# mohwald/gandtr

Hardware: AMD Instinct MI355X
Metric: images/sec generator@256^2 + descriptors/sec GeM-R101@1024^2, 1/2/4/8 MI355X (higher is better)
Workload: dtype f16c; 1 GPU; cyclegan ResnetGenerator 9-block (InstanceNorm) forward, synthetic 3x256x256, random-init weights; batch_per_gpu=64, global_batch=64, parallelism=dp1

## Files before the change

gandtr_amd/csrc/conv3x3_halo_c16.hip:

```cpp
#include <cstdio>
#include <cstdlib>

#include <vector>

#ifdef GDT_C_STAMP
#define GDT_STAMP_ON
#endif
#include "conv_device.h"

#ifndef GDT_C16_ABL
#define GDT_C16_ABL 0
#endif

namespace {

constexpr int ROWB = 128;
constexpr int QROWB = 64;
constexpr int HW_ = 18, HROWS = HW_ * HW_, HROWS_PAD = 328;
constexpr int A_BYTES = HROWS_PAD * ROWB;
constexpr int Q_BYTES = HROWS_PAD * QROWB;
constexpr int STAGE_BYTES = A_BYTES + Q_BYTES;
constexpr int NORM_BYTES = 4096 + 64;
constexpr int E_OFF = 2 * STAGE_BYTES + NORM_BYTES;
constexpr size_t LDS_BYTES = 2 * (size_t)STAGE_BYTES + NORM_BYTES + 2 * HROWS_PAD;
constexpr int NT = 256, RPR = NT / 8, NR = (HROWS_PAD + RPR - 1) / RPR;
constexpr int NTAP = 9, SLOTS = NTAP * 3;
constexpr int SPR = 2;
#ifndef GDT_C16_SDIST
#define GDT_C16_SDIST 2
#endif
constexpr int SDIST = GDT_C16_SDIST;
static_assert((NR + SDIST) * SPR <= SLOTS, "halo rounds are spread over the slots of the previous chunk");

__device__ __forceinline__ void mfma16(f32x4& acc, const f16x8& a, const f16x8& b) {
    asm volatile("v_mfma_f32_16x16x32_f16 %0, %1, %2, %0" : "+a"(acc) : "v"(a), "v"(b) : "memory");
}
__device__ __forceinline__ void mfma16_mx(f32x4& acc, const v6i& a6, const v4i& b4, int sa, int sb) {
    asm volatile("v_mfma_scale_f32_16x16x128_f8f6f4 %0, %1, %2, %0, %3, %4 op_sel_hi:[0,0,0] cbsz:2 blgp:4" : "+a"(acc) : "v"(a6), "v"(b4), "v"(sa), "v"(sb) : "memory");
}
__device__ __forceinline__ float gdt_max3_abs(float a, float b, float c) {
    float m;
    asm("v_max3_f32 %0, |%1|, |%2|, |%3|" : "=v"(m) : "v"(a), "v"(b), "v"(c));
    return m;
}
__device__ __forceinline__ float gdt_max_abs(float a, float b) {
    float m;
    asm("v_max_f32_e64 %0, |%1|, |%2|" : "=v"(m) : "v"(a), "v"(b));
    return m;
}

template <int MODE>
__global__ __launch_bounds__(NT) void conv3x3_halo_c16_kernel(const ConvLaunch d, const int vblocks) {
    constexpr bool NORM = (MODE & 1) != 0, RES = (MODE & 2) != 0, WB = (MODE & 4) != 0;
    constexpr int RING = 3;
    static_assert(18 % RING == 0, "ring slot of a half-step must not depend on the chunk");
    constexpr int AW = 8, QW = 4;
    extern __shared__ __attribute__((aligned(16))) char smem[];

    const int tid = threadIdx.x, lane = tid & 63;
    const int wave = __builtin_amdgcn_readfirstlane(tid >> 6);
    const float* __restrict__ inf = (const float*)d.in;
    const float* __restrict__ resf = (const float*)d.in_res;
    float* __restrict__ wbf = (float*)d.in_out;

    const int tiles_x = d.W >> 4, tiles_y = d.H >> 4;
    const int tpi = tiles_x * tiles_y, ntm = d.N * tpi, ntn = d.CoutPad >> 8;
    auto tile_at = [&](int vb) -> GdtPatch { return gdt_patch_at(vb, vblocks, ntm, ntn, tpi, tiles_x, 16); };
    int vb = blockIdx.x;
    GdtPatch cur = tile_at(vb);
    if (!cur.valid) return;

    const int lrow = tid >> 3;
    const bool refl = d.pad_reflect != 0;
    struct Pend { float4 r0, r1, s0, s1; unsigned goff; bool ok; };
    auto load_piece = [&](const GdtPatch& ta, int chunk, int r) -> Pend {
        int lr = lrow;
        asm volatile("" : "+v"(lr));
        const int h = min(r * RPR + lr, HROWS_PAD - 1);
        int hy, hx;
        gdt_halo_yx<HW_>(h, hy, hx);
        const int q = lane & 7;
        const int iy = ta.y0 - 1 + hy, ix = ta.x0 - 1 + hx;
        const int cbyte = (chunk * 8 + q) * 32;
        int ry, rx;
        GDT_REFLECT_CLAMP(iy, ix, d.H, d.W, ry, rx)
        const bool inb = ((unsigned)iy < (unsigned)d.H) & ((unsigned)ix < (unsigned)d.W);
        Pend p;
        p.goff = (((unsigned)((ta.n * d.H + ry) * d.W + rx) << (d.lc8 + 5)) + cbyte);
        p.ok = (h < HROWS) & (inb | refl);
        p.r0 = *(const float4*)((const char*)inf + p.goff); p.r1 = *(const float4*)((const char*)inf + p.goff + 16);
        if (RES) { p.s0 = *(const float4*)((const char*)resf + p.goff); p.s1 = *(const float4*)((const char*)resf + p.goff + 16); }
        return p;
    };
    Pend pendv[SDIST];
    float* nlds = (float*)(smem + 2 * STAGE_BYTES);
    auto stage_norm = [&](const GdtPatch& ta, int slot) {
        gdt_stage_norm(nlds, slot, d.in_norm, d.Cin, ta.n, tid, NT);
    };
    float4 nf[4];
    auto load_nf = [&](int slot, int chunk) {
        if (!NORM) return;
        const float4* np4 = (const float4*)(nlds + slot * 512 + (chunk * 8 + (lane & 7)) * 16);
#pragma unroll
        for (int k = 0; k < 4; ++k) nf[k] = np4[k];
    };
    auto store_piece = [&](int stage_off, int r, const Pend& p) {
        const int row = min(r * RPR + lrow, HROWS_PAD - 1);
        int phy, phx;
        gdt_halo_yx<HW_>(row, phy, phx);
        float a[8] = {p.r0.x, p.r0.y, p.r0.z, p.r0.w, p.r1.x, p.r1.y, p.r1.z, p.r1.w};
        if (NORM) {
            const float lo = d.in_relu ? 0.f : -3.0e38f;
#pragma unroll
            for (int k = 0; k < 4; ++k) {
                const float4 v = nf[k];
                a[2 * k] = fmaxf(fmaf(a[2 * k], v.x, v.y), lo);
                a[2 * k + 1] = fmaxf(fmaf(a[2 * k + 1], v.z, v.w), lo);
            }
            if (RES) {
                a[0] += p.s0.x; a[1] += p.s0.y; a[2] += p.s0.z; a[3] += p.s0.w;
                a[4] += p.s1.x; a[5] += p.s1.y; a[6] += p.s1.z; a[7] += p.s1.w;
            }
        }
        if (WB) {
            *(float4*)((char*)wbf + p.goff) = make_float4(a[0], a[1], a[2], a[3]);
            *(float4*)((char*)wbf + p.goff + 16) = make_float4(a[4], a[5], a[6], a[7]);
        }
#pragma unroll
        for (int e = 0; e < 8; ++e) a[e] = p.ok ? a[e] : 0.f;
        const int ex = gdt_c_pixel_exp(a);
        const float lo_scale = gdt_exp2i(ex - 13), hi_scale = gdt_exp2i(ex - 2);
        unsigned ou[4], qlo = 0, qhi = 0;
        gdt_c_split<0>(a[0], a[1], lo_scale, hi_scale, ou[0], qlo, qhi);
        gdt_c_split<1>(a[2], a[3], lo_scale, hi_scale, ou[1], qlo, qhi);
        gdt_c_split<2>(a[4], a[5], lo_scale, hi_scale, ou[2], qlo, qhi);
        gdt_c_split<3>(a[6], a[7], lo_scale, hi_scale, ou[3], qlo, qhi);
        const u32x4 ov = {ou[0], ou[1], ou[2], ou[3]};
        const int q = lane & 7;
        *(f16x8*)(smem + stage_off + row * ROWB + ((q ^ ((phx >> 1) & 7)) << 4)) = __builtin_bit_cast(f16x8, ov);
        const int key2 = (phx >> 2) & 3;
        const int qo = stage_off + A_BYTES + row * QROWB + ((((q >> 2) << 1) ^ key2) << 4) + ((q & 3) << 2);
        *(unsigned*)(smem + qo) = qlo;
        *(unsigned*)(smem + (qo ^ 16)) = qhi;
        smem[E_OFF + (stage_off ? HROWS_PAD : 0) + row] = (char)(127 + ex - 13);
    };

    float sa[8];
    unsigned sou[4], sqlo = 0, sqhi = 0;
    int sex = 0;
    float slo_scale = 1.f, shi_scale = 1.f;
    int mh = 0, mt = 0, my = 0, mx = 0, ma = 0, mb = 0;
    int wrow = 0, wx = 0, wa = 0, wq = 0;
    float mu = 0.f, ml0 = 0.f, ml1 = 0.f;
    int mbits = 0;
    int gy0 = 0, gx0 = 0;
    int wes = E_OFF + HROWS_PAD;
    auto stage_micro = [&](const GdtPatch& ta, int chunk, int stage_off, int sl, int row, int g) {
        if (GDT_C16_ABL & 1) return;
        const int r = sl / SPR, mp = ((sl % SPR) * 16 + row) * 2 + g;
        const bool st = r >= SDIST && r - SDIST < NR, ld = r < NR;
        Pend& pend = pendv[r % SDIST];
        constexpr int P_NORM = 0, P_RES = P_NORM + (NORM ? 8 : 1), P_WB = P_RES + (NORM && RES ? 3 : 0), P_MASK = P_WB + (WB ? 2 : 0), P_MAX = P_MASK + 3,
                      P_DPP = P_MAX + 2, P_EXP = P_DPP + 3, P_SPLIT = P_EXP + 2, P_ADDR = P_SPLIT + 10, P_WRITE = P_ADDR + 7, P_GADDR = P_WRITE + 4,
                      P_LOAD = P_GADDR + 9, P_END = P_LOAD + (RES ? 4 : 2);
        static_assert(P_END <= SPR * 16 * 2, "a round's micro-phases fit the positions of its slot pair");
#define GDT_PIN1(a) asm volatile("" : "+v"(a))
#define GDT_PIN2(a, b) asm volatile("" : "+v"(a), "+v"(b))
#define GDT_PIN3(a, b, c) asm volatile("" : "+v"(a), "+v"(b), "+v"(c))
#define GDT_PIN4(a, b, c, e) asm volatile("" : "+v"(a), "+v"(b), "+v"(c), "+v"(e))
        auto f4 = [](float4& v, int i) -> float& { return i == 0 ? v.x : (i == 1 ? v.y : (i == 2 ? v.z : v.w)); };
        auto pr = [&](int e) -> float& { return e < 4 ? f4(pend.r0, e) : f4(pend.r1, e - 4); };
        auto ps = [&](int e) -> float& { return e < 4 ? f4(pend.s0, e) : f4(pend.s1, e - 4); };
        if (st && !NORM && mp == P_NORM) {
#pragma unroll
            for (int e = 0; e < 8; ++e) sa[e] = pr(e);
            GDT_PIN4(sa[0], sa[1], sa[2], sa[3]); GDT_PIN4(sa[4], sa[5], sa[6], sa[7]);
        }
        if (st && NORM && mp >= P_NORM && mp < P_NORM + 8) {
            const int e = mp - P_NORM;
            const float lo = d.in_relu ? 0.f : -3.0e38f;
            const float4 v = nf[e >> 1];
            float x = pr(e);
            GDT_PIN1(x);
            x = fmaxf(fmaf(x, (e & 1) ? v.z : v.x, (e & 1) ? v.w : v.y), lo);
            GDT_PIN1(x);
            sa[e] = x;
        }
        if (st && NORM && RES && mp >= P_RES && mp < P_RES + 3) {
            const int e = 3 * (mp - P_RES);
            float y0 = ps(e), y1 = ps(e + 1), y2 = ps(e + 2 < 8 ? e + 2 : e);
            if (e + 2 < 8) { GDT_PIN3(sa[e], sa[e + 1], sa[e + 2]); GDT_PIN3(y0, y1, y2); } else { GDT_PIN2(sa[e], sa[e + 1]); GDT_PIN2(y0, y1); }
            sa[e] += y0; sa[e + 1] += y1;
            if (e + 2 < 8) { sa[e + 2] += y2; GDT_PIN3(sa[e], sa[e + 1], sa[e + 2]); } else GDT_PIN2(sa[e], sa[e + 1]);
        }
        if (st && WB && mp == P_WB) {
            GDT_PIN4(sa[0], sa[1], sa[2], sa[3]);
            *(float4*)((char*)wbf + pend.goff) = make_float4(sa[0], sa[1], sa[2], sa[3]);
        }
        if (st && WB && mp == P_WB + 1) {
            GDT_PIN4(sa[4], sa[5], sa[6], sa[7]);
            *(float4*)((char*)wbf + pend.goff + 16) = make_float4(sa[4], sa[5], sa[6], sa[7]);
        }
        if (st && mp >= P_MASK && mp < P_MASK + 3) {
            const int e = 3 * (mp - P_MASK);
            if (e + 2 < 8) GDT_PIN3(sa[e], sa[e + 1], sa[e + 2]); else GDT_PIN2(sa[e], sa[e + 1]);
            sa[e] = pend.ok ? sa[e] : 0.f; sa[e + 1] = pend.ok ? sa[e + 1] : 0.f;
            if (e + 2 < 8) { sa[e + 2] = pend.ok ? sa[e + 2] : 0.f; GDT_PIN3(sa[e], sa[e + 1], sa[e + 2]); } else GDT_PIN2(sa[e], sa[e + 1]);
        }
        if (st && mp == P_MAX) {
            GDT_PIN4(sa[0], sa[1], sa[2], sa[3]); GDT_PIN1(sa[4]);
            mu = gdt_max3_abs(gdt_max3_abs(sa[0], sa[1], sa[2]), sa[3], sa[4]);
            GDT_PIN1(mu);
        }
        if (st && mp == P_MAX + 1) {
            GDT_PIN4(mu, sa[5], sa[6], sa[7]);
            mu = gdt_max_abs(gdt_max3_abs(mu, sa[5], sa[6]), sa[7]);
            mbits = __float_as_int(mu);
            sqlo = 0; sqhi = 0;
            GDT_PIN3(mbits, sqlo, sqhi);
        }
        if (st && mp >= P_DPP && mp < P_DPP + 3) {
            GDT_PIN1(mbits);
            if (mp == P_DPP) mbits = max(mbits, __builtin_amdgcn_mov_dpp(mbits, 0xB1, 0xF, 0xF, false));
            if (mp == P_DPP + 1) mbits = max(mbits, __builtin_amdgcn_mov_dpp(mbits, 0x4E, 0xF, 0xF, false));
            if (mp == P_DPP + 2) mbits = max(mbits, __builtin_amdgcn_mov_dpp(mbits, 0x141, 0xF, 0xF, false));
            GDT_PIN1(mbits);
        }
        if (st && mp == P_EXP) {
            GDT_PIN1(mbits);
            sex = min(max(mbits >> 23, 127 - 14), 127 + 15);
            GDT_PIN1(sex);
        }
        if (st && mp == P_EXP + 1) {
            GDT_PIN1(sex);
            slo_scale = __int_as_float((sex - 13) << 23); shi_scale = __int_as_float((sex - 2) << 23);
            GDT_PIN2(slo_scale, shi_scale);
        }
        if (st && mp >= P_SPLIT && mp < P_SPLIT + 10) {
            GDT_PIN4(sqlo, sqhi, ml0, ml1);
#pragma unroll
            for (int i = 2 * (mp - P_SPLIT); i < 2 * (mp - P_SPLIT) + 2; ++i) {
                const int K = i / 5, w = i - 5 * K;
                GDT_PIN2(sa[2 * K], sa[2 * K + 1]);
                if (w > 0) GDT_PIN1(sou[K]);
                if (w == 0) sou[K] = gdt_pk_f16(sa[2 * K], sa[2 * K + 1]);
                if (w == 1) asm("v_fma_mix_f32 %0, -%1, 1.0, %2 op_sel:[0,0,0] op_sel_hi:[1,0,0]" : "=v"(ml0) : "v"(sou[K]), "v"(sa[2 * K]));
                if (w == 2) asm("v_fma_mix_f32 %0, -%1, 1.0, %2 op_sel:[1,0,0] op_sel_hi:[1,0,0]" : "=v"(ml1) : "v"(sou[K]), "v"(sa[2 * K + 1]));
                if (w == 3) {
                    GDT_PIN1(shi_scale);
                    if (K == 0) sqhi = __builtin_amdgcn_cvt_scalef32_pk_fp4_f16(sqhi, __builtin_bit_cast(f16x2, sou[K]), shi_scale, 0);
                    if (K == 1) sqhi = __builtin_amdgcn_cvt_scalef32_pk_fp4_f16(sqhi, __builtin_bit_cast(f16x2, sou[K]), shi_scale, 1);
                    if (K == 2) sqhi = __builtin_amdgcn_cvt_scalef32_pk_fp4_f16(sqhi, __builtin_bit_cast(f16x2, sou[K]), shi_scale, 2);
                    if (K == 3) sqhi = __builtin_amdgcn_cvt_scalef32_pk_fp4_f16(sqhi, __builtin_bit_cast(f16x2, sou[K]), shi_scale, 3);
                }
                if (w == 4) {
                    GDT_PIN1(slo_scale);
                    if (K == 0) sqlo = __builtin_amdgcn_cvt_scalef32_pk_fp4_f32(sqlo, ml0, ml1, slo_scale, 0);
                    if (K == 1) sqlo = __builtin_amdgcn_cvt_scalef32_pk_fp4_f32(sqlo, ml0, ml1, slo_scale, 1);
                    if (K == 2) sqlo = __builtin_amdgcn_cvt_scalef32_pk_fp4_f32(sqlo, ml0, ml1, slo_scale, 2);
                    if (K == 3) sqlo = __builtin_amdgcn_cvt_scalef32_pk_fp4_f32(sqlo, ml0, ml1, slo_scale, 3);
                }
                GDT_PIN1(sou[K]);
            }
            GDT_PIN4(sqlo, sqhi, ml0, ml1);
        }
        const int q = lane & 7;
        if (st && mp == P_ADDR) {
            int lr = lrow;
            GDT_PIN1(lr);
            wrow = min((r - SDIST) * RPR + lr, HROWS_PAD - 1);
            GDT_PIN1(wrow);
        }
        if (st && mp == P_ADDR + 1) {
            GDT_PIN1(wrow);
            wx = wrow - ((wrow * (65536 / HW_ + 1)) >> 16) * HW_;
            GDT_PIN1(wx);
        }
        if (st && mp == P_ADDR + 2) {
            GDT_PIN1(wx);
            wa = q ^ ((wx >> 1) & 7);
            GDT_PIN1(wa);
        }
        if (st && mp == P_ADDR + 3) {
            GDT_PIN2(wrow, wa);
            wa = stage_off + wrow * ROWB + (wa << 4);
            GDT_PIN1(wa);
        }
        if (st && mp == P_ADDR + 4) {
            GDT_PIN1(wx);
            wx = ((q >> 2) << 1) ^ ((wx >> 2) & 3);
            GDT_PIN1(wx);
        }
        if (st && mp == P_ADDR + 5) {
            GDT_PIN1(wx);
            wq = (wx << 4) + ((q & 3) << 2);
            GDT_PIN1(wq);
        }
        if (st && mp == P_ADDR + 6) {
            GDT_PIN2(wrow, wq);
            wq = stage_off + A_BYTES + wrow * QROWB + wq;
            GDT_PIN1(wq);
        }
        if (st && mp == P_WRITE) {
            GDT_PIN1(wa); GDT_PIN4(sou[0], sou[1], sou[2], sou[3]);
            const u32x4 ov = {sou[0], sou[1], sou[2], sou[3]};
            *(f16x8*)(smem + wa) = __builtin_bit_cast(f16x8, ov);
        }
        if (st && mp == P_WRITE + 1) {
            GDT_PIN2(wq, sqlo);
            *(unsigned*)(smem + wq) = sqlo;
        }
        if (st && mp == P_WRITE + 2) {
            GDT_PIN2(wq, sqhi);
            *(unsigned*)(smem + (wq ^ 16)) = sqhi;
        }
        if (st && mp == P_WRITE + 3) {
            GDT_PIN2(wrow, sex);
            smem[wes + wrow] = (char)(sex - 13);
        }
        if (ld && mp == P_GADDR) {
            int lr = lrow;
            GDT_PIN1(lr);
            mh = min(r * RPR + lr, HROWS_PAD - 1);
            GDT_PIN1(mh);
        }
        if (ld && mp == P_GADDR + 1) {
            GDT_PIN1(mh);
            mt = (mh * (65536 / HW_ + 1)) >> 16;
            GDT_PIN2(mh, mt);
        }
        if (ld && mp == P_GADDR + 2) {
            GDT_PIN2(mh, mt);
            my = gy0 + mt; mx = gx0 + (mh - mt * HW_);
            GDT_PIN3(mh, my, mx);
        }
        if (ld && mp == P_GADDR + 3) {
            GDT_PIN3(mh, my, mx);
            const bool inb = ((unsigned)my < (unsigned)d.H) & ((unsigned)mx < (unsigned)d.W);
            pend.ok = (mh < HROWS) & (inb | refl);
        }
        if (ld && mp == P_GADDR + 4) {
            GDT_PIN1(my);
            ma = max(my, -my); mb = 2 * d.H - 2 - ma;
            GDT_PIN2(ma, mb);
        }
        if (ld && mp == P_GADDR + 5) {
            GDT_PIN2(ma, mb);
            my = min(max(min(ma, mb), 0), d.H - 1);
            GDT_PIN1(my);
        }
        if (ld && mp == P_GADDR + 6) {
            GDT_PIN1(mx);
            ma = max(mx, -mx); mb = 2 * d.W - 2 - ma;
            GDT_PIN2(ma, mb);
        }
        if (ld && mp == P_GADDR + 7) {
            GDT_PIN2(ma, mb);
            mx = min(max(min(ma, mb), 0), d.W - 1);
            GDT_PIN1(mx);
        }
        if (ld && mp == P_GADDR + 8) {
            GDT_PIN2(my, mx);
            pend.goff = (((unsigned)((ta.n * d.H + my) * d.W + mx) << (d.lc8 + 5)) + (chunk * 8 + q) * 32);
            GDT_PIN1(pend.goff);
        }
        if (ld && mp == P_LOAD) pend.r0 = *(const float4*)((const char*)inf + pend.goff);
        if (ld && mp == P_LOAD + 1) pend.r1 = *(const float4*)((const char*)inf + pend.goff + 16);
        if (ld && RES && mp == P_LOAD + 2) pend.s0 = *(const float4*)((const char*)resf + pend.goff);
        if (ld && RES && mp == P_LOAD + 3) pend.s1 = *(const float4*)((const char*)resf + pend.goff + 16);
#undef GDT_PIN1
#undef GDT_PIN2
#undef GDT_PIN3
#undef GDT_PIN4
    };

    auto wgrp = [&](int tile_n) -> long { return (long)tile_n * 4 + wave; };
    const int nms = d.Kpad >> 6, cin64 = d.Cin >> 6;
    f16x8 bw[RING][4];
    constexpr int BQ_MFMA = (GDT_C16_ABL & 64) ? 1 : 0;
    v6i bq[1 + BQ_MFMA][4];
    v4i bqs[1 + BQ_MFMA];
    auto lane_bytes = [&](int per_lane) -> unsigned {
        unsigned v = lane * per_lane;
        asm volatile("" : "+v"(v));
        return v;
    };
    unsigned lo16 = lane_bytes(16), lo8 = lane_bytes(8), lo4 = lane_bytes(4);
    constexpr long WREC = 15360;
    auto load_bw = [&](int rs, int cb, int tile_n, long ks) {
        const char* wb = (const char*)d.w_c16 + (unsigned)(((tile_n * 4 + wave) * nms + (int)(ks >> 1)) * (int)WREC + (int)(ks & 1) * 4096);
        bw[rs][cb] = *(const f16x8*)(wb + lo16 + cb * 1024);
    };
    auto load_bq_part = [&](int set, int part, int tile_n, long ms) {
        const long f0 = (GDT_C16_ABL & 128) ? 0 : wgrp(tile_n) * nms + ms;
        const char* rec = (const char*)d.w_c16 + (unsigned)((int)f0 * (int)WREC);
        const int cb = part >> 1;
        if (part == 8) bqs[set] = *(const v4i*)(rec + 14336 + lo16);
        else if ((part & 1) == 0) {
            const v4i qa = *(const v4i*)(rec + 8192 + lo16 + cb * 1024);
            bq[set][cb] = __builtin_shufflevector(__builtin_shufflevector(qa, qa, 0, 1, 2, 3, -1, -1), bq[set][cb], 0, 1, 2, 3, 10, 11);
        } else {
            const v2i qb = *(const v2i*)(rec + 12288 + lo8 + cb * 512);
            bq[set][cb] = __builtin_shufflevector(bq[set][cb], __builtin_shufflevector(qb, qb, 0, 1, -1, -1, -1, -1), 0, 1, 2, 3, 6, 7);
        }
    };

    const int fn = lane & 15, fg = lane >> 4;
    const int px = fn < 4 ? 2 * fn : (fn < 12 ? 2 * (fn - 4) + 1 : 2 * (fn - 8));
    int vt[3], vq[3];
#pragma unroll
    for (int tx = 0; tx < 3; ++tx) {
        vt[tx] = px * ROWB + ((fg ^ (((px + tx) >> 1) & 7)) << 4);
        vq[tx] = A_BYTES + px * QROWB + ((fg ^ (((px + tx) >> 2) & 3)) << 4);
    }
    auto a_frag = [&](int pb, int ty, int tx, int s) -> f16x8 {
        return *(const f16x8*)(smem + (vt[tx] ^ (s << 6)) + ((pb + ty) * HW_ + tx) * ROWB);
    };
    auto a_qfrag = [&](int pb, int ty, int tx) -> v4i {
        return *(const v4i*)(smem + vq[tx] + ((pb + ty) * HW_ + tx) * QROWB);
    };
    int ve = E_OFF + px;
    auto a_efrag = [&](int pb, int ty, int tx) -> int {
        return *(const unsigned char*)(smem + ve + (pb + ty) * HW_ + tx);
    };
    auto flip_stage = [&](int delta) {
        ve += delta > 0 ? HROWS_PAD : -HROWS_PAD;
        wes -= delta > 0 ? HROWS_PAD : -HROWS_PAD;
#pragma unroll
        for (int k = 0; k < 3; ++k) { vt[k] += delta; vq[k] += delta; }
    };
    const int a_scale_off = (fg & 1) ? GDT_C_HI_SCALE_OFF : 0;
    constexpr bool AE_PRE = !(GDT_C16_ABL & (2 | 8));

    const int nchunks = d.Cin >> 6;
#pragma unroll
    for (int u = 0; u < RING - 1; ++u)
#pragma unroll
        for (int cb = 0; cb < 4; ++cb) load_bw(u, cb, cur.tile_n, u);
    if (NORM) {
        stage_norm(cur, 0);
        __syncthreads();
    }
    load_nf(0, 0);
#pragma unroll
    for (int r = 0; r < NR; ++r) store_piece(0, r, load_piece(cur, 0, r));
    __syncthreads();
#pragma unroll
    for (int k = 0; k < SDIST; ++k) pendv[k] = load_piece(cur, 0, 0);

    f16x8 afr[AW];
    v4i aq[QW];
    int ae[QW];
    if (GDT_C16_ABL & 8) { for (int i = 0; i < QW; ++i) { aq[i] = a_qfrag(i, 0, 0); ae[i] = a_efrag(i, 0, 0); } }
    if (GDT_C16_ABL & (16 | 64)) { for (int st = 0; st < 1 + BQ_MFMA; ++st) for (int part = 0; part < 9; ++part) load_bq_part(st, part, cur.tile_n, 0); }
#pragma unroll
    for (int i = 0; i < AW; ++i) afr[i] = a_frag(i, 0, 0, 0);

    int so = 0;
    int slot = 0;
#ifdef GDT_C_STAMP
    unsigned long long st_body = 0, st_cbar = 0, st_tbar = 0, st_epi = 0, st_t = __builtin_amdgcn_s_memtime(), st_n = 0;
    const unsigned long long st_begin = st_t;
#endif
    for (;;) {
        const GdtPatch nxt = tile_at(vb + gridDim.x);
        f32x4 acc[16][4];
#pragma unroll
        for (int i = 0; i < 16; ++i)
#pragma unroll
            for (int j = 0; j < 4; ++j)
#pragma unroll
                for (int e = 0; e < 4; ++e) acc[i][j][e] = 0.f;

        for (int c = 0; c < nchunks; ++c) {
            const bool last = c + 1 == nchunks;
            const bool to_next = last && nxt.valid;
            const GdtPatch sta = to_next ? nxt : cur;
            const int sc = last ? 0 : c + 1, sslot = to_next ? slot ^ 1 : slot;
            if (NORM && nxt.valid && c == nchunks - 2) stage_norm(nxt, slot ^ 1);
            load_nf(sslot, sc);
            lo16 = lane_bytes(16); lo8 = lane_bytes(8); lo4 = lane_bytes(4);
            auto ks_of = [&](int u) -> long { return u < 18 ? (long)(((u >> 1) * cin64 + c) * 2 + (u & 1)) : (long)(sc * 2 + (u - 18)); };
            auto tn_of = [&](int u) -> int { return (u >= 18 && last) ? nxt.tile_n : cur.tile_n; };
            gy0 = sta.y0 - 1; gx0 = sta.x0 - 1;
            asm volatile("" : "+s"(gy0), "+s"(gx0));
            __builtin_amdgcn_sched_barrier(0);
#pragma unroll
            for (int t = 0; t < NTAP; ++t) {
                const int ty = t / 3, tx = t - ty * 3;
                const int nty = (t + 1) / 3, ntx = (t + 1) - nty * 3;
#pragma unroll
                for (int s = 0; s < 2; ++s) {
                    const int u = 2 * t + s;
#pragma unroll
                    for (int pb = 0; pb < 16; ++pb) {
#pragma unroll
                        for (int cb = 0; cb < 4; ++cb) {
                            mfma16(acc[pb][cb], bw[u % RING][cb], afr[pb % AW]);
                            if (cb == 0) {
                                if (AE_PRE && s == 1 && pb == 15) { asm volatile("" : "+v"(ae[0])); ae[0] += a_scale_off; asm volatile("" : "+v"(ae[0])); }
                                if (!(GDT_C16_ABL & 4) && (pb & 3) == 2) load_bw((u + RING - 1) % RING, pb >> 2, tn_of(u + RING - 1), ks_of(u + RING - 1));
                                if (!(GDT_C16_ABL & (2 | 16)) && (pb & 1) == 1 && (s == 0 || pb == 1)) load_bq_part(0, s == 0 ? pb >> 1 : 8, cur.tile_n, (long)(t * cin64 + c));
                            } else if (cb < 3) {
                                stage_micro(sta, sc, STAGE_BYTES - so, 3 * t + s, pb, cb - 1);
                            } else {
                                if (pb + AW < 16) afr[pb % AW] = a_frag(pb + AW, ty, tx, s);
                                else if (s == 0) afr[pb % AW] = a_frag(pb + AW - 16, ty, tx, 1);
                                else if (t < NTAP - 1) afr[pb % AW] = a_frag(pb + AW - 16, nty, ntx, 0);
                                if (!(GDT_C16_ABL & (2 | 8)) && s == 1 && pb >= 16 - QW) { aq[pb - (16 - QW)] = a_qfrag(pb - (16 - QW), ty, tx); ae[pb - (16 - QW)] = a_efrag(pb - (16 - QW), ty, tx); }
                            }
                            __builtin_amdgcn_sched_barrier(0);
                        }
                    }
                }
#pragma unroll
                for (int pb = 0; pb < 16; ++pb) {
#pragma unroll
                    for (int cb = 0; cb < 4; ++cb) {
                        if (!(GDT_C16_ABL & 2)) {
                            mfma16_mx(acc[pb][cb], bq[BQ_MFMA][cb], aq[pb % QW], bqs[BQ_MFMA][cb], AE_PRE ? ae[pb % QW] : ae[pb % QW] + a_scale_off);
                            if (cb == 0 && AE_PRE && pb + 1 < 16) { asm volatile("" : "+v"(ae[(pb + 1) % QW])); ae[(pb + 1) % QW] += a_scale_off; asm volatile("" : "+v"(ae[(pb + 1) % QW])); }
                            if (cb == 3 && !(GDT_C16_ABL & 8) && pb + QW < 16) { aq[pb % QW] = a_qfrag(pb + QW, ty, tx); ae[pb % QW] = a_efrag(pb + QW, ty, tx); }
                        }
                        if (cb == 1 || cb == 2) stage_micro(sta, sc, STAGE_BYTES - so, 3 * t + 2, pb, cb - 1);
                        __builtin_amdgcn_sched_barrier(0);
                    }
                }
            }
            if (GDT_C16_ABL & 64) {
#pragma unroll
                for (int cb = 0; cb < 4; ++cb) asm volatile("" :: "v"(bq[0][cb]));
                asm volatile("" :: "v"(bqs[0]));
            }
            GDT_STAMP(st_body)
            if (!last) {
                asm volatile("s_waitcnt lgkmcnt(0)" ::: "memory");
                __builtin_amdgcn_s_barrier();
                asm volatile("" ::: "memory");
                GDT_STAMP(st_cbar)
                flip_stage(STAGE_BYTES - 2 * so);
                so = STAGE_BYTES - so;
#pragma unroll
                for (int i = 0; i < AW; ++i) afr[i] = a_frag(i, 0, 0, 0);
            }
        }

        asm volatile("s_waitcnt lgkmcnt(0)" ::: "memory");
        __builtin_amdgcn_s_barrier();
        asm volatile("" ::: "memory");
        GDT_STAMP(st_tbar)
        const int so_next = STAGE_BYTES - so;

        {
            float* __restrict__ outp = (float*)d.out;
            const float* __restrict__ resp = (const float*)d.res;
            int lane_e = lane;
            asm volatile("" : "+v"(lane_e));
            const int n_e = lane_e & 15, g_e = lane_e >> 4;
            const int x_e = n_e < 4 ? 2 * n_e : (n_e < 12 ? 2 * (n_e - 4) + 1 : 2 * (n_e - 8));
            const int ch = cur.tile_n * 256 + wave * 64 + 4 * g_e;
            unsigned o = (unsigned)((cur.n * d.H + cur.y0) * d.W + cur.x0 + x_e) * (unsigned)d.Cout + (unsigned)ch;
            const unsigned rowstep = (unsigned)d.W * (unsigned)d.Cout;
            const bool lowhalf = n_e < 8;
            const int n_p = n_e ^ 8, x_p = n_p < 4 ? 2 * n_p : (n_p < 12 ? 2 * (n_p - 4) + 1 : 2 * (n_p - 8));
            const unsigned o_p = o + (unsigned)((x_p - x_e) * d.Cout);
            unsigned oA = (lowhalf ? o : o_p) + (lowhalf ? 0u : 16u), oB = (lowhalf ? o_p : o) + (lowhalf ? 0u : 16u);
            const float lo = d.relu ? 0.f : -__builtin_inff();
            constexpr bool EPI_RES = MODE == 0;
            const bool has_res = EPI_RES && resp != nullptr;
            float4 bv[4], s1[4], s2[4];
#pragma unroll
            for (int cb = 0; cb < 4; ++cb) {
                bv[cb] = d.bias ? *(const float4*)(d.bias + ch + cb * 16) : make_float4(0.f, 0.f, 0.f, 0.f);
                s1[cb] = make_float4(0.f, 0.f, 0.f, 0.f); s2[cb] = make_float4(0.f, 0.f, 0.f, 0.f);
            }
            float4 rcur[4], rnxt[4];
            if (has_res) {
#pragma unroll
                for (int cb = 0; cb < 4; ++cb) rcur[cb] = *(const float4*)(resp + o + cb * 16);
            }
#pragma unroll
            for (int pb = 0; pb < 16; ++pb) {
                asm volatile("" : "+v"(o));
                if (has_res && pb + 1 < 16) {
#pragma unroll
                    for (int cb = 0; cb < 4; ++cb) rnxt[cb] = *(const float4*)(resp + o + rowstep + cb * 16);
                }
                float4 tv[4];
#pragma unroll
                for (int cb = 0; cb < 4; ++cb) {
                    const f32x4& a = acc[pb][cb];
                    float4 t = make_float4(a[0] + bv[cb].x, a[1] + bv[cb].y, a[2] + bv[cb].z, a[3] + bv[cb].w);
                    s1[cb].x += t.x; s1[cb].y += t.y; s1[cb].z += t.z; s1[cb].w += t.w;
                    s2[cb].x += t.x * t.x; s2[cb].y += t.y * t.y; s2[cb].z += t.z * t.z; s2[cb].w += t.w * t.w;
                    if (has_res) { t.x += rcur[cb].x; t.y += rcur[cb].y; t.z += rcur[cb].z; t.w += rcur[cb].w; }
                    t.x = fmaxf(t.x, lo); t.y = fmaxf(t.y, lo); t.z = fmaxf(t.z, lo); t.w = fmaxf(t.w, lo);
                    tv[cb] = t;
                }
                if (GDT_C16_ABL & 256) {
#pragma unroll
                    for (int cb = 0; cb < 4; ++cb) asm volatile("" :: "v"(tv[cb].x), "v"(tv[cb].y), "v"(tv[cb].z), "v"(tv[cb].w));
                } else {
                    auto ror8 = [](float v) -> float { return __builtin_bit_cast(float, __builtin_amdgcn_update_dpp(0, __builtin_bit_cast(int, v), 0x128, 0xf, 0xf, false)); };
#pragma unroll
                    for (int p2 = 0; p2 < 2; ++p2) {
                        const float4 t0 = tv[2 * p2], t1 = tv[2 * p2 + 1];
                        const float rx = ror8(lowhalf ? t1.x : t0.x), ry = ror8(lowhalf ? t1.y : t0.y), rz = ror8(lowhalf ? t1.z : t0.z), rw = ror8(lowhalf ? t1.w : t0.w);
                        *(float4*)(outp + oA + p2 * 32) = make_float4(lowhalf ? t0.x : rx, lowhalf ? t0.y : ry, lowhalf ? t0.z : rz, lowhalf ? t0.w : rw);
                        *(float4*)(outp + oB + p2 * 32) = make_float4(lowhalf ? rx : t1.x, lowhalf ? ry : t1.y, lowhalf ? rz : t1.z, lowhalf ? rw : t1.w);
                    }
                    oA += rowstep; oB += rowstep;
                }
                o += rowstep;
                if (has_res) {
#pragma unroll
                    for (int cb = 0; cb < 4; ++cb) rcur[cb] = rnxt[cb];
                }
            }
            if (d.stats) {
                auto merge = [](float v) -> float {
                    v += __builtin_bit_cast(float, __builtin_amdgcn_update_dpp(0, __builtin_bit_cast(int, v), 0x128, 0xf, 0xf, false));
                    v += __builtin_bit_cast(float, __builtin_amdgcn_update_dpp(0, __builtin_bit_cast(int, v), 0x124, 0xf, 0xf, false));
                    v += __builtin_bit_cast(float, __builtin_amdgcn_update_dpp(0, __builtin_bit_cast(int, v), 0x122, 0xf, 0xf, false));
                    v += __builtin_bit_cast(float, __builtin_amdgcn_update_dpp(0, __builtin_bit_cast(int, v), 0x121, 0xf, 0xf, false));
                    return v;
                };
#pragma unroll
                for (int cb = 0; cb < 4; ++cb) {
                    s1[cb].x = merge(s1[cb].x); s1[cb].y = merge(s1[cb].y); s1[cb].z = merge(s1[cb].z); s1[cb].w = merge(s1[cb].w);
                    s2[cb].x = merge(s2[cb].x); s2[cb].y = merge(s2[cb].y); s2[cb].z = merge(s2[cb].z); s2[cb].w = merge(s2[cb].w);
                }
                if (n_e == 0) {
                    float* dst = d.stats + ((long)(d.stats_tile_base + cur.tile_m * 2) * 2) * d.Cout + ch;
#pragma unroll
                    for (int cb = 0; cb < 4; ++cb) {
                        *(float4*)(dst + cb * 16) = s1[cb];
                        *(float4*)(dst + d.Cout + cb * 16) = s2[cb];
                        *(float4*)(dst + 2l * d.Cout + cb * 16) = make_float4(0.f, 0.f, 0.f, 0.f);
                        *(float4*)(dst + 3l * d.Cout + cb * 16) = make_float4(0.f, 0.f, 0.f, 0.f);
                    }
                }
            }
        }
#ifdef GDT_C_STAMP
        asm volatile("s_waitcnt vmcnt(0)" ::: "memory");
        GDT_STAMP(st_epi)
        ++st_n;
#endif
        if (!nxt.valid) break;
        cur = nxt; vb += gridDim.x; slot ^= 1;
        flip_stage(so_next - so);
        so = so_next;
#pragma unroll
        for (int i = 0; i < AW; ++i) afr[i] = a_frag(i, 0, 0, 0);
    }
#ifdef GDT_C_STAMP
    if (lane == 0 && d.stamp_out) {
        unsigned long long* o = d.stamp_out + ((long)blockIdx.x * 4 + wave) * 8;
        o[0] = st_body; o[1] = st_cbar; o[2] = st_tbar; o[3] = st_epi; o[4] = __builtin_amdgcn_s_memtime() - st_begin; o[5] = st_n;
    }
#endif
}

template <int MODE>
int launch_c16(const ConvLaunch& d, hipStream_t stream) {
    using K = GdtKernel<conv3x3_halo_c16_kernel<MODE>, (int)LDS_BYTES>;
    int cus = 0;
    GDT_CHECK(K::figure(cus));
    const int vblocks = gdt_grid_for_tiles(d.N * (d.W >> 4) * (d.H >> 4), d.CoutPad >> 8);
    const int grid = vblocks < cus ? vblocks : cus;
#ifdef GDT_C_STAMP
    static unsigned long long* stamp_buf = nullptr;
    static int stamp_calls = 0;
    ConvLaunch ds = d;
    if (!stamp_buf) GDT_CHECK_HIP(hipMalloc((void**)&stamp_buf, (size_t)cus * 4 * 8 * sizeof(unsigned long long)));
    GDT_CHECK_HIP(hipMemsetAsync(stamp_buf, 0, (size_t)cus * 4 * 8 * sizeof(unsigned long long), stream));
    ds.stamp_out = stamp_buf;
    GDT_CHECK(K::launch(grid, NT, stream, ds, vblocks));
    if (++stamp_calls % 200 < 20) {
        GDT_CHECK_HIP(hipStreamSynchronize(stream));
        std::vector<unsigned long long> h((size_t)grid * 4 * 8);
        GDT_CHECK_HIP(hipMemcpy(h.data(), stamp_buf, h.size() * sizeof(unsigned long long), hipMemcpyDeviceToHost));
        double s[6] = {0, 0, 0, 0, 0, 0};
        for (size_t w = 0; w < (size_t)grid * 4; ++w) for (int k = 0; k < 6; ++k) s[k] += (double)h[w * 8 + k];
        const double nw = grid * 4.0, nt = s[5] / nw;
        fprintf(stderr, "[c stamp] MODE %d FORM 16 BN 256 waves 4: tiles/wave %.1f; per tile: chunk bodies %.0f, chunk barriers %.0f, tile barrier %.0f, epilogue %.0f cycles; total per wave %.0f\n",
                MODE, nt, s[0] / nw / nt, s[1] / nw / nt, s[2] / nw / nt, s[3] / nw / nt, s[4] / nw);
    }
    return GDT_OK;
#else
    return K::launch(grid, NT, stream, d, vblocks);
#endif
}

GDT_KNOB_LATCHED(knob_mode, "GDT_CONV_HALO_C16", 1)

}

bool gdt_conv_halo_c16_eligible(const ConvLaunch& d) {
    if (knob_mode() == 0 || !d.w_c16) return false;
    if (!gdt_conv_halo_c_eligible(d) || gdt_conv_halo_c_columns(d) != 256) return false;
    if ((d.H & 15) || (d.W & 15) || d.Cout != d.CoutPad || (d.Cout & 255)) return false;
    if (d.res && d.in_norm) return false;
    if ((unsigned long long)(d.CoutPad >> 6) * (unsigned long long)(d.Kpad >> 6) * 15360ull >= (1ull << 32)) return false;
    return true;
}

int gdt_launch_conv_halo_c16(const ConvLaunch& d, hipStream_t stream) {
    switch (gdt_fold_mode(d)) {
        case 0: return launch_c16<0>(d, stream);
        case 1: return launch_c16<1>(d, stream);
        case 3: return launch_c16<3>(d, stream);
        case 5: return launch_c16<5>(d, stream);
        default: return launch_c16<7>(d, stream);
    }
}
```

Before: 6092 images/s.

## Schedule staging micro-phases with compile-time placement table per slot-pair type

Replaces the fixed linear mapping of staging micro-phases onto MFMA issue slots with a constexpr-generated program that places each phase according to dependencies and which rows may take vector-memory ops, varying across three cycling pair types. The tap loop becomes a compile-time integer_sequence expansion so the table lookups fold to constants. The MX weight record offset is computed once per tap and kept in a scalar register instead of recomputed per partial load. It aims to spread global loads and dependent ALU work more evenly between MFMAs to reduce stalls, at the cost of more complex scheduling logic and possibly larger code.

```diff
diff --git a/gandtr_amd/csrc/conv3x3_halo_c16.hip b/gandtr_amd/csrc/conv3x3_halo_c16.hip
--- a/gandtr_amd/csrc/conv3x3_halo_c16.hip
+++ b/gandtr_amd/csrc/conv3x3_halo_c16.hip
@@ -1,6 +1,8 @@
 #include <cstdio>
 #include <cstdlib>
 
+#include <type_traits>
+#include <utility>
 #include <vector>
 
 #ifdef GDT_C_STAMP
@@ -48,6 +50,57 @@
     asm("v_max_f32_e64 %0, |%1|, |%2|" : "=v"(m) : "v"(a), "v"(b));
     return m;
 }
+
+template <int MODE> struct C16Ids {
+    static constexpr bool NORM = (MODE & 1) != 0, RES = (MODE & 2) != 0, WB = (MODE & 4) != 0;
+    static constexpr int P_NORM = 0, P_RES = P_NORM + (NORM ? 8 : 1), P_WB = P_RES + (NORM && RES ? 3 : 0), P_MASK = P_WB + (WB ? 2 : 0), P_MAX = P_MASK + 3,
+                         P_DPP = P_MAX + 2, P_EXP = P_DPP + 3, P_SPLIT = P_EXP + 2, P_ADDR = P_SPLIT + 10, P_WRITE = P_ADDR + 7, P_GADDR = P_WRITE + 4,
+                         P_LOAD = P_GADDR + 9, P_END = P_LOAD + (RES ? 4 : 2);
+};
+constexpr int C16_NPOS = SPR * 16 * 2;
+struct C16Prog { signed char at[3][C16_NPOS]; bool complete; };
+constexpr bool c16_row_takes_vmem(int kind, int row) {
+    return kind == 2 || (kind == 0 ? (row & 3) == 0 : ((row & 3) != 2 && row != 1));
+}
+template <int MODE> constexpr C16Prog c16_make_prog() {
+    using P = C16Ids<MODE>;
+    static_assert(SPR == 2, "pair types: two slots of three cycling kinds");
+    C16Prog pg{};
+    pg.complete = true;
+    for (int ty = 0; ty < 3; ++ty) {
+        bool placed[P::P_END] = {};
+        int vrow = -1;
+        for (int p = 0; p < C16_NPOS; ++p) {
+            const int prow = p >> 1, kind = (2 * ty + (prow >> 4)) % 3;
+            const bool vmem_ok = c16_row_takes_vmem(kind, prow & 15) && prow != vrow;
+            int pick = -1;
+            for (int pass = 0; pass < 4 && pick < 0; ++pass)
+                for (int id = 0; id < P::P_END && pick < 0; ++id) {
+                    if (placed[id]) continue;
+                    const bool vmem = (P::WB && id >= P::P_WB && id < P::P_MASK) || id >= P::P_LOAD;
+                    const bool lside = id >= P::P_GADDR, addr = id >= P::P_ADDR && id < P::P_WRITE;
+                    if ((vmem ? pass != 0 : (lside ? pass != (P::NORM && placed[P::P_MASK + 2] ? 1 : 3) : pass != 2)) || (vmem && !vmem_ok)) continue;
+                    bool ready = true;
+                    if (addr) ready = id == P::P_ADDR || placed[id - 1];
+                    else if (lside) ready = (id == P::P_GADDR || placed[id - 1]) && (id != P::P_GADDR + 3 || placed[P::P_MASK + 2]);
+                    else if (id == P::P_WRITE) ready = placed[P::P_ADDR - 1] && placed[P::P_WRITE - 1];
+                    else if (P::WB && id == P::P_MASK) ready = placed[P::P_WB];
+                    else if (P::WB && id == P::P_MASK + 1) ready = placed[P::P_MASK] && placed[P::P_WB + 1];
+                    else ready = id == 0 || placed[id - 1];
+                    if (ready) pick = id;
+                }
+            pg.at[ty][p] = (signed char)pick;
+            if (pick >= 0) {
+                placed[pick] = true;
+                if ((P::WB && pick >= P::P_WB && pick < P::P_MASK) || pick >= P::P_LOAD) vrow = prow;
+            }
+        }
+        for (int id = 0; id < P::P_END; ++id) pg.complete = pg.complete && placed[id];
+    }
+    return pg;
+}
+template <int MODE> constexpr C16Prog c16_prog = c16_make_prog<MODE>();
+template <class F, int... T> __device__ __forceinline__ void c16_each_tap(F&& f, std::integer_sequence<int, T...>) { (f(std::integral_constant<int, T>{}), ...); }
 
 template <int MODE>
 __global__ __launch_bounds__(NT) void conv3x3_halo_c16_kernel(const ConvLaunch d, const int vblocks) {
@@ -155,15 +208,16 @@
     int mbits = 0;
     int gy0 = 0, gx0 = 0;
     int wes = E_OFF + HROWS_PAD;
-    auto stage_micro = [&](const GdtPatch& ta, int chunk, int stage_off, int sl, int row, int g) {
+    auto stage_micro = [&](const GdtPatch& ta, int chunk, int stage_off, int sl, int row, int g) __attribute__((always_inline)) {
         if (GDT_C16_ABL & 1) return;
-        const int r = sl / SPR, mp = ((sl % SPR) * 16 + row) * 2 + g;
+        const int r = sl / SPR;
+        const int mp = c16_prog<MODE>.at[r % 3][((sl % SPR) * 16 + row) * 2 + g];
         const bool st = r >= SDIST && r - SDIST < NR, ld = r < NR;
         Pend& pend = pendv[r % SDIST];
-        constexpr int P_NORM = 0, P_RES = P_NORM + (NORM ? 8 : 1), P_WB = P_RES + (NORM && RES ? 3 : 0), P_MASK = P_WB + (WB ? 2 : 0), P_MAX = P_MASK + 3,
-                      P_DPP = P_MAX + 2, P_EXP = P_DPP + 3, P_SPLIT = P_EXP + 2, P_ADDR = P_SPLIT + 10, P_WRITE = P_ADDR + 7, P_GADDR = P_WRITE + 4,
-                      P_LOAD = P_GADDR + 9, P_END = P_LOAD + (RES ? 4 : 2);
-        static_assert(P_END <= SPR * 16 * 2, "a round's micro-phases fit the positions of its slot pair");
+        using P = C16Ids<MODE>;
+        constexpr int P_NORM = P::P_NORM, P_RES = P::P_RES, P_WB = P::P_WB, P_MASK = P::P_MASK, P_MAX = P::P_MAX, P_DPP = P::P_DPP, P_EXP = P::P_EXP,
+                      P_SPLIT = P::P_SPLIT, P_ADDR = P::P_ADDR, P_WRITE = P::P_WRITE, P_GADDR = P::P_GADDR, P_LOAD = P::P_LOAD;
+        static_assert(c16_prog<MODE>.complete, "a round's micro-phases fit the positions of its slot pair, in all three pair types");
 #define GDT_PIN1(a) asm volatile("" : "+v"(a))
 #define GDT_PIN2(a, b) asm volatile("" : "+v"(a), "+v"(b))
 #define GDT_PIN3(a, b, c) asm volatile("" : "+v"(a), "+v"(b), "+v"(c))
@@ -387,13 +441,18 @@
     };
     unsigned lo16 = lane_bytes(16), lo8 = lane_bytes(8), lo4 = lane_bytes(4);
     constexpr long WREC = 15360;
-    auto load_bw = [&](int rs, int cb, int tile_n, long ks) {
+    auto load_bw = [&](int rs, int cb, int tile_n, long ks) __attribute__((always_inline)) {
         const char* wb = (const char*)d.w_c16 + (unsigned)(((tile_n * 4 + wave) * nms + (int)(ks >> 1)) * (int)WREC + (int)(ks & 1) * 4096);
         bw[rs][cb] = *(const f16x8*)(wb + lo16 + cb * 1024);
     };
-    auto load_bq_part = [&](int set, int part, int tile_n, long ms) {
+    auto bq_record = [&](int tile_n, long ms) -> int {
         const long f0 = (GDT_C16_ABL & 128) ? 0 : wgrp(tile_n) * nms + ms;
-        const char* rec = (const char*)d.w_c16 + (unsigned)((int)f0 * (int)WREC);
+        int off = (int)f0 * (int)WREC;
+        asm volatile("" : "+s"(off));
+        return off;
+    };
+    auto load_bq_part = [&](int set, int part, int recoff) __attribute__((always_inline)) {
+        const char* rec = (const char*)d.w_c16 + (unsigned)recoff;
         const int cb = part >> 1;
         if (part == 8) bqs[set] = *(const v4i*)(rec + 14336 + lo16);
         else if ((part & 1) == 0) {
@@ -452,7 +511,7 @@
     v4i aq[QW];
     int ae[QW];
     if (GDT_C16_ABL & 8) { for (int i = 0; i < QW; ++i) { aq[i] = a_qfrag(i, 0, 0); ae[i] = a_efrag(i, 0, 0); } }
-    if (GDT_C16_ABL & (16 | 64)) { for (int st = 0; st < 1 + BQ_MFMA; ++st) for (int part = 0; part < 9; ++part) load_bq_part(st, part, cur.tile_n, 0); }
+    if (GDT_C16_ABL & (16 | 64)) { for (int st = 0; st < 1 + BQ_MFMA; ++st) for (int part = 0; part < 9; ++part) load_bq_part(st, part, bq_record(cur.tile_n, 0)); }
 #pragma unroll
     for (int i = 0; i < AW; ++i) afr[i] = a_frag(i, 0, 0, 0);
 
@@ -485,10 +544,11 @@
             gy0 = sta.y0 - 1; gx0 = sta.x0 - 1;
             asm volatile("" : "+s"(gy0), "+s"(gx0));
             __builtin_amdgcn_sched_barrier(0);
-#pragma unroll
-            for (int t = 0; t < NTAP; ++t) {
-                const int ty = t / 3, tx = t - ty * 3;
-                const int nty = (t + 1) / 3, ntx = (t + 1) - nty * 3;
+            c16_each_tap([&](auto tap) __attribute__((always_inline)) {
+                constexpr int t = decltype(tap)::value;
+                constexpr int ty = t / 3, tx = t - ty * 3;
+                constexpr int nty = (t + 1) / 3, ntx = (t + 1) - nty * 3;
+                int mxrec = 0;
 #pragma unroll
                 for (int s = 0; s < 2; ++s) {
                     const int u = 2 * t + s;
@@ -498,9 +558,10 @@
                         for (int cb = 0; cb < 4; ++cb) {
                             mfma16(acc[pb][cb], bw[u % RING][cb], afr[pb % AW]);
                             if (cb == 0) {
+                                if (s == 0 && pb == 0) mxrec = bq_record(cur.tile_n, (long)(t * cin64 + c));
                                 if (AE_PRE && s == 1 && pb == 15) { asm volatile("" : "+v"(ae[0])); ae[0] += a_scale_off; asm volatile("" : "+v"(ae[0])); }
                                 if (!(GDT_C16_ABL & 4) && (pb & 3) == 2) load_bw((u + RING - 1) % RING, pb >> 2, tn_of(u + RING - 1), ks_of(u + RING - 1));
-                                if (!(GDT_C16_ABL & (2 | 16)) && (pb & 1) == 1 && (s == 0 || pb == 1)) load_bq_part(0, s == 0 ? pb >> 1 : 8, cur.tile_n, (long)(t * cin64 + c));
+                                if (!(GDT_C16_ABL & (2 | 16)) && (pb & 1) == 1 && (s == 0 || pb == 1)) load_bq_part(0, s == 0 ? pb >> 1 : 8, mxrec);
                             } else if (cb < 3) {
                                 stage_micro(sta, sc, STAGE_BYTES - so, 3 * t + s, pb, cb - 1);
                             } else {
@@ -526,7 +587,7 @@
                         __builtin_amdgcn_sched_barrier(0);
                     }
                 }
-            }
+            }, std::make_integer_sequence<int, NTAP>{});
             if (GDT_C16_ABL & 64) {
 #pragma unroll
                 for (int cb = 0; cb < 4; ++cb) asm volatile("" :: "v"(bq[0][cb]));
```

Result: no change. 6131 images/s, median of 6 (+0.6%).
